# SUNGBEOMCHOI/Rubiks-Cube-Solver

Hardware: AMD Instinct MI355X
Metric: cube-move steps/sec, 3x3x3 batch 4M; HBM GB/s vs roofline at 1/2/4/8 GPU (higher is better)
Workload: dtype u8; 1 GPU; 3x3x3 apply_move + solved flag, 4194304 cubes/GPU/launch x 1 GPU(s), u8 SoA [54][N], ping-pong; configs[1] shape at the metric's batch 4M; cubes_per_gpu=4194304, total_cubes=4194304, parallelism=1 independent ranks, stream_id = rank, no collective, distinct_devices=1, pci_bus_id=0000:0d:00

## Files before the change

rubiks-cube-solver_amd/csrc/rc_tree.cpp:

```cpp
#include "../../include/rubiktree.h"

#include <omp.h>

#include <cmath>
#include <cstring>
#include <string>
#include <unordered_map>
#include <vector>

namespace {

constexpr int kMaxA = 12, kMaxSlots = 20;

struct Mt {
    uint32_t mt[624];
    uint32_t idx;
    uint32_t next() {
        if (idx >= 624) {
            for (int k = 0; k < 624; ++k) {
                const uint32_t y = (mt[k] & 0x80000000u) | (mt[(k + 1) % 624] & 0x7fffffffu);
                mt[k] = mt[(k + 397) % 624] ^ (y >> 1) ^ ((y & 1u) ? 0x9908b0dfu : 0u);
            }
            idx = 0;
        }
        uint32_t y = mt[idx++];
        y ^= y >> 11; y ^= (y << 7) & 0x9d2c5680u; y ^= (y << 15) & 0xefc60000u; y ^= y >> 18;
        return y;
    }
    int below(int n) {
        int k = 0;
        while ((n >> k) != 0) ++k;
        uint32_t r = next() >> (32 - k);
        while ((int)r >= n) r = next() >> (32 - k);
        return (int)r;
    }
};

struct Node {
    float policy[kMaxA];
    double value[kMaxA];
    double vloss[kMaxA];
    int32_t visits[kMaxA];
    int32_t child[kMaxA];
    uint8_t key[kMaxA][kMaxSlots];
    uint8_t done[kMaxA];
};

struct Tree {
    std::vector<Node> nodes;
    std::unordered_map<std::string, int32_t> index;
    std::vector<std::pair<int32_t, uint8_t>> trail;
    std::string leaf_key;
    std::vector<uint8_t> solution;
    bool solved = false, active = false;
    int32_t sims = 0;
};

}

struct rc_tree {
    int n, A, slots;
    double c, vl, vmin;
    bool shared = false, have_rng = false;
    int threads = 1;
    std::vector<Tree> trees;
    std::vector<Mt> rng;
    int last_depth = 0;
};

namespace {

int puct_best(const Node &nd, int A, double c) {
    long total = 0;
    for (int i = 0; i < A; ++i) total += nd.visits[i];
    const double root = std::sqrt((double)total);
    const float c32 = (float)c;
    int arg = 0;
    float best = 0.f;
    for (int i = 0; i < A; ++i) {
        const float cp = c32 * nd.policy[i];
        const float x = (float)(root / (double)(1 + nd.visits[i]));
        const float u = cp * x;
        const float uw = u + (float)nd.value[i];
        const float s = uw - (float)nd.vloss[i];
        if (i == 0 || s > best) { best = s; arg = i; }
    }
    return arg;
}

int32_t descend_from(rc_tree *t, Tree &tr, int32_t cur, Mt *gen) {
    while (cur >= 0) {
        Node &nd = tr.nodes[(size_t)cur];
        long total = 0;
        for (int i = 0; i < t->A; ++i) total += nd.visits[i];
        if (total == 0 && gen == nullptr) return cur;
        const int a = total == 0 ? gen->below(t->A) : puct_best(nd, t->A, t->c);
        nd.vloss[a] += t->vl;
        tr.trail.emplace_back(cur, (uint8_t)a);
        int32_t nxt = nd.child[a];
        if (nxt < 0) {
            const std::string key(reinterpret_cast<const char *>(nd.key[a]), (size_t)t->slots);
            const auto it = tr.index.find(key);
            if (it != tr.index.end()) nxt = nd.child[a] = it->second;
            else tr.leaf_key = key;
        }
        cur = nxt;
    }
    return -1;
}

int32_t descend_begin(rc_tree *t, int r, Mt *gen) {
    Tree &tr = t->trees[(size_t)r];
    tr.trail.clear();
    tr.leaf_key.clear();
    tr.active = !tr.solved;
    if (!tr.active) return -1;
    ++tr.sims;
    return descend_from(t, tr, tr.nodes.empty() ? -1 : 0, gen);
}

}

#ifndef RC_SRC_HASH
#define RC_SRC_HASH unhashed
#endif
#define RC_STR2(x) #x
#define RC_STR(x) RC_STR2(x)
static const char k_build_id[] = "rc-build-id:" RC_STR(RC_SRC_HASH);

extern "C" {

const char *rc_tree_build_id(void) { return k_build_id + 12; }

rc_tree *rc_tree_create(int n_roots, int n_actions, int n_slots, double cpuct, double virtual_loss, double value_min) {
    if (n_roots <= 0 || n_actions <= 0 || n_actions > kMaxA || n_slots <= 0 || n_slots > kMaxSlots) return nullptr;
    rc_tree *t = new rc_tree;
    t->n = n_roots; t->A = n_actions; t->slots = n_slots;
    t->c = cpuct; t->vl = virtual_loss; t->vmin = value_min;
    t->trees.resize((size_t)n_roots);
    return t;
}

void rc_tree_destroy(rc_tree *t) { delete t; }

int rc_tree_set_threads(rc_tree *t, int threads) {
    if (!t || threads < 1) return -1;
    const int mx = omp_get_max_threads();
    t->threads = threads < mx ? threads : mx;
    return t->threads;
}

int rc_tree_set_rng(rc_tree *t, int shared, const uint32_t *states) {
    if (!t || !states) return -1;
    t->shared = shared != 0;
    t->rng.resize(t->shared ? 1 : (size_t)t->n);
    for (size_t g = 0; g < t->rng.size(); ++g) {
        memcpy(t->rng[g].mt, states + g * 625, 624 * sizeof(uint32_t));
        t->rng[g].idx = states[g * 625 + 624];
        if (t->rng[g].idx > 624) return -1;
    }
    t->have_rng = true;
    return 0;
}

int rc_tree_get_rng(const rc_tree *t, uint32_t *states) {
    if (!t || !states || !t->have_rng) return -1;
    for (size_t g = 0; g < t->rng.size(); ++g) {
        memcpy(states + g * 625, t->rng[g].mt, 624 * sizeof(uint32_t));
        states[g * 625 + 624] = t->rng[g].idx;
    }
    return 0;
}

int rc_tree_select(rc_tree *t) {
    if (!t || !t->have_rng) return -1;
    if (t->shared) {
        std::vector<int32_t> resume((size_t)t->n);
#pragma omp parallel for schedule(dynamic, 16) num_threads(t->threads)
        for (int r = 0; r < t->n; ++r) resume[(size_t)r] = descend_begin(t, r, nullptr);
        for (int r = 0; r < t->n; ++r)
            if (resume[(size_t)r] >= 0) descend_from(t, t->trees[(size_t)r], resume[(size_t)r], &t->rng[0]);
    } else {
#pragma omp parallel for schedule(dynamic, 16) num_threads(t->threads)
        for (int r = 0; r < t->n; ++r) descend_begin(t, r, &t->rng[(size_t)r]);
    }
    int depth = 0;
    for (const Tree &tr : t->trees)
        if (tr.active && (int)tr.trail.size() > depth) depth = (int)tr.trail.size();
    t->last_depth = depth;
    return depth;
}

int rc_tree_paths(const rc_tree *t, uint8_t *paths, int pitch) {
    if (!t || !paths || pitch < t->last_depth) return -1;
    for (int r = 0; r < t->n; ++r) {
        uint8_t *row = paths + (size_t)r * (size_t)pitch;
        memset(row, t->A, (size_t)pitch);
        const Tree &tr = t->trees[(size_t)r];
        if (tr.active)
            for (size_t d = 0; d < tr.trail.size(); ++d) row[d] = tr.trail[d].second;
    }
    return 0;
}

int rc_tree_update(rc_tree *t, const uint8_t *leaf_code, const uint8_t *child_code, const uint8_t *solved, const float *value,
                   const float *policy) {
    if (!t || !leaf_code || !child_code || !solved || !value || !policy) return -1;
    const int A = t->A, SL = t->slots;
#pragma omp parallel for schedule(dynamic, 16) num_threads(t->threads)
    for (int r = 0; r < t->n; ++r) {
        Tree &tr = t->trees[(size_t)r];
        if (!tr.active) continue;
        Node nd;
        bool any = false;
        int first = -1;
        for (int a = 0; a < A; ++a) {
            nd.policy[a] = policy[(size_t)r * A + a];
            nd.value[a] = t->vmin;
            nd.vloss[a] = 0.0;
            nd.visits[a] = 0;
            nd.child[a] = -1;
            memcpy(nd.key[a], child_code + ((size_t)r * A + a) * SL, (size_t)SL);
            nd.done[a] = solved[(size_t)r * A + a] != 0;
            if (nd.done[a] && !any) { any = true; first = a; }
        }
        const int32_t id = (int32_t)tr.nodes.size();
        tr.nodes.push_back(nd);
        const std::string own(reinterpret_cast<const char *>(leaf_code + (size_t)r * SL), (size_t)SL);
        if (id == 0) tr.index.emplace(own, 0);
        else tr.index.emplace(tr.leaf_key, id);
        const float v = value[r];
        for (auto it = tr.trail.rbegin(); it != tr.trail.rend(); ++it) {
            Node &p = tr.nodes[(size_t)it->first];
            const int a = it->second;
            if ((double)v > p.value[a]) p.value[a] = (double)v;
            p.vloss[a] -= 150.0;
            p.visits[a] += 1;
        }
        if (any) {
            tr.solution.clear();
            for (const auto &pa : tr.trail) tr.solution.push_back(pa.second);
            tr.solution.push_back((uint8_t)first);
            tr.solved = true;
        }
        tr.active = false;
    }
    int done = 0;
    for (const Tree &tr : t->trees) done += tr.solved;
    return done;
}

int rc_tree_solution(const rc_tree *t, int root, uint8_t *out, int cap) {
    if (!t || root < 0 || root >= t->n) return -2;
    const Tree &tr = t->trees[(size_t)root];
    if (!tr.solved) return -1;
    const int len = (int)tr.solution.size();
    if (out)
        for (int i = 0; i < len && i < cap; ++i) out[i] = tr.solution[(size_t)i];
    return len;
}

int rc_tree_sims_used(const rc_tree *t, int32_t *out) {
    if (!t || !out) return -1;
    for (int r = 0; r < t->n; ++r) out[r] = t->trees[(size_t)r].sims;
    return 0;
}

int rc_tree_root_stats(const rc_tree *t, int root, int32_t *visits, double *values) {
    if (!t || root < 0 || root >= t->n) return -1;
    const Tree &tr = t->trees[(size_t)root];
    for (int a = 0; a < t->A; ++a) {
        if (visits) visits[a] = tr.nodes.empty() ? 0 : tr.nodes[0].visits[a];
        if (values) values[a] = tr.nodes.empty() ? -1.0 : tr.nodes[0].value[a];
    }
    return (int)tr.nodes.size();
}

}
```

Before: 64.96 billion steps/s.

## Rework MCTS tree storage with open-addressing index and grouped prefetched descent

Replaces the string-keyed unordered_map with a fixed-key linear-probing hash table and stores nodes in chunked, cache-line-aligned blocks. Hot edge fields (precomputed c*policy, visits, float value/vloss mirrors) are packed first. Descent interleaves eight trees per thread with software prefetch, and backup prefetches trail nodes ahead. Path emission is parallelised. This aims to cut host-side pointer chasing and allocation cost, at the price of keeping duplicated float/double accumulators that must stay in sync.

```diff
diff --git a/rubiks-cube-solver_amd/csrc/rc_tree.cpp b/rubiks-cube-solver_amd/csrc/rc_tree.cpp
--- a/rubiks-cube-solver_amd/csrc/rc_tree.cpp
+++ b/rubiks-cube-solver_amd/csrc/rc_tree.cpp
@@ -3,14 +3,19 @@
 #include <omp.h>
 
 #include <cmath>
+#include <cstddef>
 #include <cstring>
-#include <string>
-#include <unordered_map>
+#include <memory>
+#include <utility>
 #include <vector>
 
 namespace {
 
 constexpr int kMaxA = 12, kMaxSlots = 20;
+constexpr int kChunkShift = 5, kChunk = 1 << kChunkShift;
+constexpr int kGroup = 8;
+constexpr int kAhead = 8;
+constexpr int32_t kPause = -2;
 
 struct Mt {
     uint32_t mt[624];
@@ -36,24 +41,105 @@
     }
 };
 
-struct Node {
-    float policy[kMaxA];
-    double value[kMaxA];
-    double vloss[kMaxA];
-    int32_t visits[kMaxA];
+struct Key {
+    uint8_t b[kMaxSlots];
+};
+
+inline bool same_key(const Key &x, const Key &y) { return memcmp(x.b, y.b, kMaxSlots) == 0; }
+
+inline uint32_t hash_key(const Key &k) {
+    uint64_t a, b;
+    uint32_t c;
+    memcpy(&a, k.b, 8); memcpy(&b, k.b + 8, 8); memcpy(&c, k.b + 16, 4);
+    uint64_t h = a * 0x9E3779B97F4A7C15ull;
+    h ^= h >> 32; h += b; h *= 0xBF58476D1CE4E5B9ull;
+    h ^= h >> 29; h += c; h *= 0x94D049BB133111EBull;
+    return (uint32_t)(h >> 32);
+}
+
+struct Edge {
+    float cp;
+    int32_t n;
+    float wf, lf;
+};
+
+struct Acc {
+    double w, l;
+};
+
+struct alignas(64) Node {
+    Edge e[kMaxA];
     int32_t child[kMaxA];
-    uint8_t key[kMaxA][kMaxSlots];
-    uint8_t done[kMaxA];
+    int32_t pad[4];
+    Acc acc[kMaxA];
+    Key key[kMaxA];
+};
+static_assert(sizeof(Edge) == 16 && sizeof(Acc) == 16 && offsetof(Node, child) == 192 && offsetof(Node, acc) == 256, "a descent reads the first four lines of a node");
+
+inline void prefetch_node(const Node *p) {
+    const char *c = reinterpret_cast<const char *>(p);
+    __builtin_prefetch(c); __builtin_prefetch(c + 64); __builtin_prefetch(c + 128); __builtin_prefetch(c + 192);
+}
+
+inline int32_t total_visits(const Node &nd, int A) {
+    int32_t total = 0;
+    for (int i = 0; i < A; ++i) total += nd.e[i].n;
+    return total;
+}
+
+struct Index {
+    struct Slot { Key key; int32_t id; };
+    std::vector<Slot> slot;
+    uint32_t used = 0;
+
+    int32_t find(const Key &k) const {
+        if (slot.empty()) return -1;
+        const uint32_t mask = (uint32_t)slot.size() - 1;
+        for (uint32_t i = hash_key(k) & mask;; i = (i + 1) & mask) {
+            const Slot &s = slot[i];
+            if (s.id < 0) return -1;
+            if (same_key(s.key, k)) return s.id;
+        }
+    }
+    void place(const Key &k, int32_t id) {
+        const uint32_t mask = (uint32_t)slot.size() - 1;
+        uint32_t i = hash_key(k) & mask;
+        while (slot[i].id >= 0) i = (i + 1) & mask;
+        slot[i].key = k; slot[i].id = id;
+    }
+    void insert_if_absent(const Key &k, int32_t id) {
+        if (find(k) >= 0) return;
+        if (2 * (used + 1) > slot.size()) {
+            std::vector<Slot> old;
+            old.swap(slot);
+            Slot empty;
+            memset(&empty, 0, sizeof(empty));
+            empty.id = -1;
+            slot.assign(old.empty() ? 64 : 2 * old.size(), empty);
+            for (const Slot &s : old)
+                if (s.id >= 0) place(s.key, s.id);
+        }
+        place(k, id);
+        ++used;
+    }
 };
 
 struct Tree {
-    std::vector<Node> nodes;
-    std::unordered_map<std::string, int32_t> index;
+    std::vector<std::unique_ptr<Node[]>> chunks;
+    int32_t count = 0;
+    Index index;
     std::vector<std::pair<int32_t, uint8_t>> trail;
-    std::string leaf_key;
+    Key leaf_key;
+    bool have_leaf = false;
     std::vector<uint8_t> solution;
     bool solved = false, active = false;
     int32_t sims = 0;
+
+    Node &node(int32_t i) const { return chunks[(size_t)(i >> kChunkShift)][(size_t)(i & (kChunk - 1))]; }
+    Node &append() {
+        if ((count & (kChunk - 1)) == 0) chunks.emplace_back(new Node[kChunk]);
+        return node(count++);
+    }
 };
 
 }
@@ -65,58 +151,87 @@
     int threads = 1;
     std::vector<Tree> trees;
     std::vector<Mt> rng;
+    std::vector<int32_t> resume;
     int last_depth = 0;
 };
 
 namespace {
 
-int puct_best(const Node &nd, int A, double c) {
-    long total = 0;
-    for (int i = 0; i < A; ++i) total += nd.visits[i];
+int puct_best(const Node &nd, int A, int32_t total) {
     const double root = std::sqrt((double)total);
-    const float c32 = (float)c;
+    const float root32 = (float)root;
     int arg = 0;
     float best = 0.f;
     for (int i = 0; i < A; ++i) {
-        const float cp = c32 * nd.policy[i];
-        const float x = (float)(root / (double)(1 + nd.visits[i]));
-        const float u = cp * x;
-        const float uw = u + (float)nd.value[i];
-        const float s = uw - (float)nd.vloss[i];
+        const Edge &e = nd.e[i];
+        const float x = e.n == 0 ? root32 : (float)(root / (double)(1 + e.n));
+        const float u = e.cp * x;
+        const float uw = u + e.wf;
+        const float s = uw - e.lf;
         if (i == 0 || s > best) { best = s; arg = i; }
     }
     return arg;
 }
 
-int32_t descend_from(rc_tree *t, Tree &tr, int32_t cur, Mt *gen) {
-    while (cur >= 0) {
-        Node &nd = tr.nodes[(size_t)cur];
-        long total = 0;
-        for (int i = 0; i < t->A; ++i) total += nd.visits[i];
-        if (total == 0 && gen == nullptr) return cur;
-        const int a = total == 0 ? gen->below(t->A) : puct_best(nd, t->A, t->c);
-        nd.vloss[a] += t->vl;
-        tr.trail.emplace_back(cur, (uint8_t)a);
-        int32_t nxt = nd.child[a];
-        if (nxt < 0) {
-            const std::string key(reinterpret_cast<const char *>(nd.key[a]), (size_t)t->slots);
-            const auto it = tr.index.find(key);
-            if (it != tr.index.end()) nxt = nd.child[a] = it->second;
-            else tr.leaf_key = key;
-        }
-        cur = nxt;
-    }
-    return -1;
-}
-
-int32_t descend_begin(rc_tree *t, int r, Mt *gen) {
-    Tree &tr = t->trees[(size_t)r];
-    tr.trail.clear();
-    tr.leaf_key.clear();
-    tr.active = !tr.solved;
-    if (!tr.active) return -1;
-    ++tr.sims;
-    return descend_from(t, tr, tr.nodes.empty() ? -1 : 0, gen);
+inline int32_t descend_step(const rc_tree *t, Tree &tr, int32_t cur, Mt *gen) {
+    Node &nd = tr.node(cur);
+    const int32_t total = total_visits(nd, t->A);
+    if (total == 0 && gen == nullptr) return kPause;
+    const int a = total == 0 ? gen->below(t->A) : puct_best(nd, t->A, total);
+    nd.acc[a].l += t->vl;
+    nd.e[a].lf = (float)nd.acc[a].l;
+    tr.trail.emplace_back(cur, (uint8_t)a);
+    int32_t nxt = nd.child[a];
+    if (nxt < 0) {
+        nxt = tr.index.find(nd.key[a]);
+        if (nxt >= 0) nd.child[a] = nxt;
+        else { tr.leaf_key = nd.key[a]; tr.have_leaf = true; }
+    }
+    return nxt;
+}
+
+void descend_from(const rc_tree *t, Tree &tr, int32_t cur, Mt *gen) {
+    while (cur >= 0) cur = descend_step(t, tr, cur, gen);
+}
+
+int descend_group(rc_tree *t, int r0, int cnt, int32_t *resume) {
+    int32_t cur[kGroup];
+    int live[kGroup], nlive = 0;
+    for (int k = 0; k < cnt; ++k) {
+        Tree &tr = t->trees[(size_t)(r0 + k)];
+        tr.trail.clear();
+        tr.have_leaf = false;
+        tr.active = !tr.solved;
+        if (resume) resume[r0 + k] = -1;
+        if (!tr.active) continue;
+        ++tr.sims;
+        if (tr.count == 0) continue;
+        cur[k] = 0;
+        live[nlive++] = k;
+        prefetch_node(&tr.node(0));
+    }
+    while (nlive > 0) {
+        int m = 0;
+        for (int j = 0; j < nlive; ++j) {
+            const int k = live[j];
+            Tree &tr = t->trees[(size_t)(r0 + k)];
+            const int32_t nxt = descend_step(t, tr, cur[k], resume ? nullptr : &t->rng[(size_t)(r0 + k)]);
+            if (nxt >= 0) {
+                prefetch_node(&tr.node(nxt));
+                cur[k] = nxt;
+                live[m++] = k;
+            } else if (nxt == kPause) {
+                resume[r0 + k] = cur[k];
+            }
+        }
+        nlive = m;
+    }
+    int depth = 0;
+    for (int k = 0; k < cnt; ++k) {
+        const Tree &tr = t->trees[(size_t)(r0 + k)];
+        if (tr.active && (int)tr.trail.size() > depth) depth = (int)tr.trail.size();
+    }
+    return depth;
 }
 
 }
@@ -174,31 +289,39 @@
 
 int rc_tree_select(rc_tree *t) {
     if (!t || !t->have_rng) return -1;
+    const int n = t->n, groups = (n + kGroup - 1) / kGroup;
+    int32_t *resume = nullptr;
     if (t->shared) {
-        std::vector<int32_t> resume((size_t)t->n);
-#pragma omp parallel for schedule(dynamic, 16) num_threads(t->threads)
-        for (int r = 0; r < t->n; ++r) resume[(size_t)r] = descend_begin(t, r, nullptr);
-        for (int r = 0; r < t->n; ++r)
-            if (resume[(size_t)r] >= 0) descend_from(t, t->trees[(size_t)r], resume[(size_t)r], &t->rng[0]);
-    } else {
-#pragma omp parallel for schedule(dynamic, 16) num_threads(t->threads)
-        for (int r = 0; r < t->n; ++r) descend_begin(t, r, &t->rng[(size_t)r]);
+        t->resume.resize((size_t)n);
+        resume = t->resume.data();
     }
     int depth = 0;
-    for (const Tree &tr : t->trees)
-        if (tr.active && (int)tr.trail.size() > depth) depth = (int)tr.trail.size();
+#pragma omp parallel for schedule(dynamic, 2) num_threads(t->threads) reduction(max : depth)
+    for (int g = 0; g < groups; ++g) {
+        const int r0 = g * kGroup;
+        const int d = descend_group(t, r0, n - r0 < kGroup ? n - r0 : kGroup, resume);
+        if (d > depth) depth = d;
+    }
+    if (resume)
+        for (int r = 0; r < n; ++r) {
+            if (resume[r] < 0) continue;
+            Tree &tr = t->trees[(size_t)r];
+            descend_from(t, tr, resume[r], &t->rng[0]);
+            if ((int)tr.trail.size() > depth) depth = (int)tr.trail.size();
+        }
     t->last_depth = depth;
     return depth;
 }
 
 int rc_tree_paths(const rc_tree *t, uint8_t *paths, int pitch) {
     if (!t || !paths || pitch < t->last_depth) return -1;
+#pragma omp parallel for schedule(static) num_threads(t->threads)
     for (int r = 0; r < t->n; ++r) {
         uint8_t *row = paths + (size_t)r * (size_t)pitch;
-        memset(row, t->A, (size_t)pitch);
         const Tree &tr = t->trees[(size_t)r];
-        if (tr.active)
-            for (size_t d = 0; d < tr.trail.size(); ++d) row[d] = tr.trail[d].second;
+        const size_t len = tr.active ? tr.trail.size() : 0;
+        for (size_t d = 0; d < len; ++d) row[d] = tr.trail[d].second;
+        memset(row + len, t->A, (size_t)pitch - len);
     }
     return 0;
 }
@@ -207,46 +330,61 @@
                    const float *policy) {
     if (!t || !leaf_code || !child_code || !solved || !value || !policy) return -1;
     const int A = t->A, SL = t->slots;
-#pragma omp parallel for schedule(dynamic, 16) num_threads(t->threads)
+    const float c32 = (float)t->c, vmin32 = (float)t->vmin;
+    int done = 0;
+#pragma omp parallel for schedule(dynamic, 16) num_threads(t->threads) reduction(+ : done)
     for (int r = 0; r < t->n; ++r) {
         Tree &tr = t->trees[(size_t)r];
-        if (!tr.active) continue;
-        Node nd;
-        bool any = false;
+        if (!tr.active) { done += tr.solved; continue; }
+        const std::pair<int32_t, uint8_t> *trail = tr.trail.data();
+        const int len = (int)tr.trail.size();
+        const auto prefetch_trail = [&](int i) {
+            const Node *p = &tr.node(trail[i].first);
+            __builtin_prefetch(&p->e[trail[i].second], 1); __builtin_prefetch(&p->acc[trail[i].second], 1);
+        };
+        for (int i = len - 1; i >= 0 && i >= len - kAhead; --i) prefetch_trail(i);
+        const int32_t id = tr.count;
+        Node &nd = tr.append();
         int first = -1;
         for (int a = 0; a < A; ++a) {
-            nd.policy[a] = policy[(size_t)r * A + a];
-            nd.value[a] = t->vmin;
-            nd.vloss[a] = 0.0;
-            nd.visits[a] = 0;
+            nd.e[a].cp = c32 * policy[(size_t)r * A + a];
+            nd.e[a].n = 0;
+            nd.e[a].wf = vmin32;
+            nd.e[a].lf = 0.f;
+            nd.acc[a].w = t->vmin;
+            nd.acc[a].l = 0.0;
             nd.child[a] = -1;
-            memcpy(nd.key[a], child_code + ((size_t)r * A + a) * SL, (size_t)SL);
-            nd.done[a] = solved[(size_t)r * A + a] != 0;
-            if (nd.done[a] && !any) { any = true; first = a; }
-        }
-        const int32_t id = (int32_t)tr.nodes.size();
-        tr.nodes.push_back(nd);
-        const std::string own(reinterpret_cast<const char *>(leaf_code + (size_t)r * SL), (size_t)SL);
-        if (id == 0) tr.index.emplace(own, 0);
-        else tr.index.emplace(tr.leaf_key, id);
+            memset(nd.key[a].b, 0, kMaxSlots);
+            memcpy(nd.key[a].b, child_code + ((size_t)r * A + a) * SL, (size_t)SL);
+            if (first < 0 && solved[(size_t)r * A + a] != 0) first = a;
+        }
+        if (id == 0) {
+            Key own;
+            memset(own.b, 0, kMaxSlots);
+            memcpy(own.b, leaf_code + (size_t)r * SL, (size_t)SL);
+            tr.index.insert_if_absent(own, 0);
+        } else if (tr.have_leaf) {
+            tr.index.insert_if_absent(tr.leaf_key, id);
+        }
         const float v = value[r];
-        for (auto it = tr.trail.rbegin(); it != tr.trail.rend(); ++it) {
-            Node &p = tr.nodes[(size_t)it->first];
-            const int a = it->second;
-            if ((double)v > p.value[a]) p.value[a] = (double)v;
-            p.vloss[a] -= 150.0;
-            p.visits[a] += 1;
-        }
-        if (any) {
+        for (int i = len - 1; i >= 0; --i) {
+            if (i >= kAhead) prefetch_trail(i - kAhead);
+            Node &p = tr.node(trail[i].first);
+            const int a = trail[i].second;
+            if ((double)v > p.acc[a].w) { p.acc[a].w = (double)v; p.e[a].wf = v; }
+            p.acc[a].l -= 150.0;
+            p.e[a].lf = (float)p.acc[a].l;
+            p.e[a].n += 1;
+        }
+        if (first >= 0) {
             tr.solution.clear();
-            for (const auto &pa : tr.trail) tr.solution.push_back(pa.second);
+            for (int i = 0; i < len; ++i) tr.solution.push_back(trail[i].second);
             tr.solution.push_back((uint8_t)first);
             tr.solved = true;
         }
         tr.active = false;
-    }
-    int done = 0;
-    for (const Tree &tr : t->trees) done += tr.solved;
+        done += tr.solved;
+    }
     return done;
 }
 
@@ -270,10 +408,10 @@
     if (!t || root < 0 || root >= t->n) return -1;
     const Tree &tr = t->trees[(size_t)root];
     for (int a = 0; a < t->A; ++a) {
-        if (visits) visits[a] = tr.nodes.empty() ? 0 : tr.nodes[0].visits[a];
-        if (values) values[a] = tr.nodes.empty() ? -1.0 : tr.nodes[0].value[a];
-    }
-    return (int)tr.nodes.size();
-}
-
-}
+        if (visits) visits[a] = tr.count == 0 ? 0 : tr.node(0).e[a].n;
+        if (values) values[a] = tr.count == 0 ? -1.0 : tr.node(0).acc[a].w;
+    }
+    return tr.count;
+}
+
+}
```

Result: no change. 64.93 billion steps/s (-0.0%).
